# enoche/MMRec

Hardware: NVIDIA H100
Metric: graph-prop edges/sec (+ full-catalog scored-items/sec in extra) @ d=64 (higher is better)
Workload: dtype f32

## Files before the change

### mmrec_b200/csrc/score_cf.cu

```cuda
#include <climits>
#include <cstdio>
#include <cstdlib>

#include "batch_mask.cuh"
#include "select.cuh"
#include "tc_common.cuh"

namespace mmrec {

using namespace tc;

constexpr int CF_TILE = 128;
constexpr int CF_CONSUMER_WARPS = 8;
constexpr int CF_THREADS = 32 * CF_CONSUMER_WARPS + 32;
constexpr int CF_MAX_STAGES = 10;
constexpr int CF_CAP = 512;
constexpr int CF_EX_SLOTS = 128;
constexpr float CF_EPS = 1.125f / 1024.f;
constexpr float CF_EPS_SUB = 1.0f / 16777216.f;

struct CfSmem {
    uint32_t a, slab0, slab, bars, total;
    int stages;
};
__host__ __device__ inline CfSmem cf_smem(int KP) {
    CfSmem L;
    L.a = 0;
    L.slab0 = 2 * CF_TILE * KP * 2;
    const uint32_t slab = CF_TILE * KP * 2;
    L.slab = slab;
    L.stages = (int)((226u * 1024u - L.slab0 - 300u) / slab);
    if (L.stages > CF_MAX_STAGES) L.stages = CF_MAX_STAGES;
    L.bars = L.slab0 + L.stages * slab;
    L.total = L.bars + 32 * 8;
    return L;
}
enum { CB_AFULL = 0, CB_AFREE = 1, CB_FULL = 2, CB_EMPTY = 2 + CF_MAX_STAGES, CB_END = 2 + 2 * CF_MAX_STAGES };

struct CfParams {
    const char* Upk;
    const char* Ipk;
    int KP, n_it;
    int64_t B, n_items, n_units;
    float* gmax; int G, gw;
    const float* thr; uint4* bitmap;
    int dbg;
};

__device__ __forceinline__ void cf_producer(const CfParams& p, const CfSmem& L, uint32_t sbase, int64_t u0, int64_t u1) {
    const uint32_t bar = sbase + L.bars;
    const uint32_t a_bytes = 2 * CF_TILE * p.KP * 2;
    const uint32_t piece = L.slab < 16384u ? L.slab : 16384u;
    int64_t pair = u0 / p.n_it;
    int it = (int)(u0 - pair * p.n_it);
    bool new_pair = true;
    uint32_t a_cnt = 0, slot = 0, ph = 1;
    for (int64_t u = u0; u < u1; ++u) {
        if (new_pair) {
            if (a_cnt > 0) mbar_wait(bar + CB_AFREE * 8, (a_cnt - 1) & 1);
            mbar_expect_tx(bar + CB_AFULL * 8, a_bytes);
            const char* src = p.Upk + pair * (int64_t)a_bytes;
            for (uint32_t o = 0; o < a_bytes; o += 16384) bulk_g2s(sbase + L.a + o, src + o, 16384, bar + CB_AFULL * 8);
            ++a_cnt;
            new_pair = false;
        }
        const char* src = p.Ipk + (int64_t)it * L.slab;
        const uint32_t fb = bar + (CB_FULL + slot) * 8;
        mbar_wait(bar + (CB_EMPTY + slot) * 8, ph);
        if (p.dbg & 16) {
            mbar_arrive(fb);
        } else {
            mbar_expect_tx(fb, L.slab);
            const uint32_t dst = sbase + L.slab0 + slot * L.slab;
            for (uint32_t o = 0; o < L.slab; o += piece) bulk_g2s(dst + o, src + o, piece, fb);
        }
        if (++slot == (uint32_t)L.stages) { slot = 0; ph ^= 1; }
        if (++it == p.n_it) { it = 0; ++pair; new_pair = true; }
    }
}

template <int PASS, int GPT>
__device__ __forceinline__ void cf_consumer(const CfParams& p, const CfSmem& L, uint32_t sbase, int64_t u0, int64_t u1, int h) {
    const uint32_t bar = sbase + L.bars;
    constexpr uint32_t LBO = (CF_TILE / 8) * 128, SBO = 128;
    const int ksteps = p.KP / 16;
    const uint32_t half_bytes = CF_TILE * p.KP * 2;
    const int t = threadIdx.x & 127, w = t >> 5, lane = t & 31, q = lane & 3;
    const uint64_t a_desc0 = smem_desc(sbase + L.a + h * half_bytes, LBO, SBO), a_desc1 = smem_desc(sbase + L.a + h * half_bytes + 1024, LBO, SBO);
    const uint64_t b_desc0 = smem_desc(sbase + L.slab0, LBO, SBO);
    const uint64_t kstep = (2 * LBO) >> 4;
    const uint64_t slab_step = L.slab >> 4;
    float acc0[64], acc1[64];
#pragma unroll
    for (int i = 0; i < 64; ++i) { acc0[i] = 0.f; acc1[i] = 0.f; }
    int64_t pair = u0 / p.n_it;
    int it = (int)(u0 - pair * p.n_it);
    bool new_pair = true, live = false;
    uint32_t a_cnt = 0, slot = 0, ph = 0;
    uint64_t bd_slot = b_desc0;
    int64_t row0 = 0;
    float thr[4];
    for (int64_t u = u0; u < u1; ++u) {
        if (new_pair) {
            mbar_wait(bar + CB_AFULL * 8, a_cnt & 1);
            ++a_cnt;
            const int64_t base = pair * (2 * CF_TILE) + h * CF_TILE;
            live = base < p.B;
            row0 = base + 16 * w + (lane >> 2);
#pragma unroll
            for (int r = 0; r < 4; ++r) {
                const int64_t rr = row0 + 64 * (r >> 1) + 8 * (r & 1);
                if (PASS == 2) thr[r] = rr < p.B ? __ldg(p.thr + rr) : INFINITY;
            }
            new_pair = false;
        }
        mbar_wait(bar + (CB_FULL + slot) * 8, ph);
        if (live && !(p.dbg & 2)) {
            uint64_t ad0 = a_desc0, ad1 = a_desc1, bd = bd_slot;
            wgmma_fence();
#pragma unroll 4
            for (int j = 0; j < ksteps; ++j) {
                wgmma_f16<CF_TILE>(acc0, ad0, bd, j ? 1u : 0u);
                wgmma_f16<CF_TILE>(acc1, ad1, bd, j ? 1u : 0u);
                ad0 += kstep; ad1 += kstep; bd += kstep;
            }
            wgmma_commit();
            wgmma_wait<0>();
            wgmma_fence_regs(acc0);
            wgmma_fence_regs(acc1);
        }
        warp_arrive(bar + (CB_EMPTY + slot) * 8);
        bd_slot += slab_step;
        if (++slot == (uint32_t)L.stages) { slot = 0; ph ^= 1; bd_slot = b_desc0; }
        const int cur_it = it;
        if (++it == p.n_it) { it = 0; ++pair; new_pair = true; }
        if (new_pair || u + 1 == u1) warp_arrive(bar + CB_AFREE * 8);
        if (!live) continue;
        const int n_valid = (int)(p.n_items - (int64_t)cur_it * CF_TILE);
#pragma unroll
        for (int r = 0; r < 4; ++r) {
            const float* acc = r < 2 ? acc0 : acc1;
            const int e2 = r & 1;
            const int64_t row = row0 + 64 * (r >> 1) + 8 * e2;
            auto val = [&](int j, int e) {
                const float v = acc[4 * j + 2 * e2 + e];
                return 8 * j + 2 * q + e < n_valid ? v : -INFINITY;
            };
            if (PASS == 1) {
                group_max_store<GPT>(r < 2 ? acc0 : acc1, e2, q, n_valid, row, p.B, [&] { return p.gmax + row * p.G + (int64_t)cur_it * GPT; });
            } else {
                uint32_t wd[4] = {0u, 0u, 0u, 0u};
#pragma unroll
                for (int j = 0; j < 16; ++j)
#pragma unroll
                    for (int e = 0; e < 2; ++e)
                        if (!(__float_as_uint(val(j, e) - thr[r]) >> 31)) wd[j >> 2] |= 1u << (31 - (8 * (j & 3) + 2 * q + e));
#pragma unroll
                for (int b = 0; b < 4; ++b) {
                    wd[b] |= __shfl_xor_sync(0xffffffffu, wd[b], 1);
                    wd[b] |= __shfl_xor_sync(0xffffffffu, wd[b], 2);
                }
                if (q == r && row < p.B) p.bitmap[row * p.n_it + cur_it] = make_uint4(wd[0], wd[1], wd[2], wd[3]);
            }
        }
    }
}

template <int PASS, int GPT>
__global__ void __launch_bounds__(CF_THREADS, 1) cf_pass_kernel(const CfParams p) {
    extern __shared__ __align__(1024) uint8_t smem[];
    const CfSmem L = cf_smem(p.KP);
    const uint32_t sbase = smem_u32(smem);
    const int warp = threadIdx.x >> 5, lane = threadIdx.x & 31;
    const uint32_t bar = sbase + L.bars;
    if (threadIdx.x == 0) {
        mbar_init(bar + CB_AFULL * 8, 1);
        mbar_init(bar + CB_AFREE * 8, CF_CONSUMER_WARPS);
        for (int s = 0; s < CF_MAX_STAGES; ++s) {
            mbar_init(bar + (CB_FULL + s) * 8, 1);
            mbar_init(bar + (CB_EMPTY + s) * 8, CF_CONSUMER_WARPS);
        }
        mbar_fence_init();
    }
    __syncthreads();
    const int64_t u0 = (int64_t)blockIdx.x * p.n_units / gridDim.x;
    const int64_t u1 = (int64_t)(blockIdx.x + 1) * p.n_units / gridDim.x;
    if (warp == CF_CONSUMER_WARPS) {
        if (lane == 0) cf_producer(p, L, sbase, u0, u1);
    } else {
        cf_consumer<PASS, GPT>(p, L, sbase, u0, u1, warp >> 2);
    }
}

__device__ __forceinline__ void cf_pack_one(int64_t t, int64_t n_rows, const int64_t* __restrict__ idx, const float* __restrict__ E, int64_t ld,
                                            int d, int KP, const uint32_t* __restrict__ scale_src, uint4* __restrict__ out,
                                            float* __restrict__ row_norm, uint32_t* __restrict__ max_norm) {
    const int kblks = KP / 8;
    const int64_t row = t / kblks;
    const int kb = (int)(t % kblks);
    float x[8];
#pragma unroll
    for (int e = 0; e < 8; ++e) x[e] = 0.f;
    if (row < n_rows) {
        const float* src = E + (idx ? idx[row] : row) * ld;
#pragma unroll
        for (int e = 0; e < 8; ++e)
            if (kb * 8 + e < d) x[e] = __ldg(src + kb * 8 + e);
    }
    uint32_t am = 0u;
    if (!scale_src) {
#pragma unroll
        for (int e = 0; e < 8; ++e) { const uint32_t b = __float_as_uint(x[e]) & 0x7fffffffu; am = b > am ? b : am; }
        for (int o = kblks / 2; o > 0; o >>= 1) {
            const uint32_t a2 = __shfl_xor_sync(0xffffffffu, am, o);
            am = a2 > am ? a2 : am;
        }
    }
    const float sc = fp16_scale_for(scale_src ? __ldg(scale_src) : am);
    float ss = 0.f;
#pragma unroll
    for (int e = 0; e < 8; ++e) ss = fmaf(x[e] * sc, x[e] * sc, ss);
    for (int o = kblks / 2; o > 0; o >>= 1) ss += __shfl_xor_sync(0xffffffffu, ss, o);
    store_fp16x8(out, row / CF_TILE, kblks, kb, (int)(row % CF_TILE), x, sc);
    if (kb == 0 && row < n_rows) {
        const float nrm = sqrtf(ss) * (1.0f + 1e-6f);
        if (row_norm) row_norm[row] = nrm;
        if (max_norm) atomicMax(max_norm, __float_as_uint(nrm));
    }
}

__global__ void __launch_bounds__(256) cf_pack_items_kernel(int64_t n_items, const float* __restrict__ Ie, int64_t ldi, int d, int KP,
                                                            uint4* __restrict__ Ipk, uint32_t* __restrict__ header, int64_t n_threads) {
    const int64_t t = blockIdx.x * (int64_t)blockDim.x + threadIdx.x;
    if (t >= n_threads) return;
    if (t == 0) { header[1] = (uint32_t)n_items; header[2] = (uint32_t)d; header[3] = (uint32_t)KP; }
    cf_pack_one(t, n_items, nullptr, Ie, ldi, d, KP, header + 4, Ipk, nullptr, header);
}

__global__ void __launch_bounds__(256) cf_prep_kernel(int64_t mask_blocks, const BatchMask mask, int64_t nb, const int64_t* __restrict__ users,
                                                      const float* __restrict__ Ue, int64_t ldu, int d, int KP, uint4* __restrict__ Upk,
                                                      float* __restrict__ unorm, int64_t pack_threads, uint32_t* __restrict__ zero, int64_t zero_words) {
    if ((int64_t)blockIdx.x < mask_blocks) {
        mask_sorted_block(blockIdx.x, mask);
        return;
    }
    int64_t t = (blockIdx.x - mask_blocks) * (int64_t)blockDim.x + threadIdx.x;
    if (t < pack_threads) { cf_pack_one(t, nb, users, Ue, ldu, d, KP, nullptr, Upk, unorm, nullptr); return; }
    t -= pack_threads;
    if (t < zero_words) zero[t] = 0;
}

constexpr int CF_THR_BITS = 16;
template <int NV>
__device__ __forceinline__ uint32_t cf_warp_kth_coarse(const float* __restrict__ g, int G, int need, int lane) {
    uint32_t key[NV];
#pragma unroll
    for (int j = 0; j < NV; ++j) {
        const int t = j * 32 + lane;
        key[j] = t < G ? float_key(__ldg(g + t)) : 0u;
    }
    uint32_t kmax = 0u, kmin = 0xffffffffu;
#pragma unroll
    for (int j = 0; j < NV; ++j) {
        kmax = max(kmax, key[j]);
        if (j * 32 + lane < G && key[j] > 0x007fffffu) kmin = min(kmin, key[j]);
    }
    kmax = __reduce_max_sync(0xffffffffu, kmax);
    kmin = __reduce_min_sync(0xffffffffu, kmin);
    const int top = 31 - __clz((kmax ^ kmin) | (1u << (32 - CF_THR_BITS)));
    uint32_t prefix = top >= 31 ? 0u : (kmax & ~((2u << top) - 1u));
#pragma unroll 1
    for (int b = top; b >= 32 - CF_THR_BITS; --b) {
        const uint32_t cand = prefix | (1u << b);
        int cnt = 0;
#pragma unroll
        for (int j = 0; j < NV; ++j) cnt += key[j] >= cand;
        cnt = __reduce_add_sync(0xffffffffu, cnt);
        if (cnt >= need) prefix = cand;
    }
    return prefix;
}

__global__ void __launch_bounds__(256) cf_thr_kernel(int64_t nb, int G, int G_valid, int k, int d, const float* __restrict__ gmax, const float* __restrict__ unorm,
                                                     const uint32_t* __restrict__ max_norm, const int32_t* __restrict__ mask_ptr,
                                                     float* __restrict__ thr, int32_t* __restrict__ flags) {
    __shared__ RadixSmem radix_all[8];
    const int lane = threadIdx.x & 31, warp = threadIdx.x >> 5;
    const int64_t row = (int64_t)blockIdx.x * 8 + warp;
    if (row >= nb) return;
    const int need = k + (mask_ptr ? mask_ptr[row + 1] - mask_ptr[row] : 0);
    if (need > G_valid) {
        if (lane == 0) { thr[row] = INFINITY; flags[row] = 1; }
        return;
    }
    const float* g = gmax + row * G;
    uint32_t kth;
    if (G <= 16 * 32) kth = cf_warp_kth_coarse<16>(g, G, need, lane);
    else if (G <= 32 * 32) kth = cf_warp_kth_coarse<32>(g, G, need, lane);
    else {
        unsigned need_u = (unsigned)need;
        kth = radix_select<4, 32>([=](int64_t t) { return float_key(__ldg(g + t)); }, G, need_u, radix_all[warp]);
    }
    if (lane == 0) {
        const float un = unorm[row], mn = __uint_as_float(*max_norm);
        set_threshold(key_float(kth), 2.0f * (CF_EPS * un * mn + CF_EPS_SUB * sqrtf((float)d) * (un + mn + 1.0f)), thr + row, flags + row);
    }
}

__host__ __device__ constexpr int cf_lpr(int d) { return d <= 32 ? 8 : (d <= 64 ? 16 : 32); }

__device__ __forceinline__ float4 cf_load4(const float* __restrict__ row, int l, int d, bool vec_ok) {
    float4 x = make_float4(0.f, 0.f, 0.f, 0.f);
    if (vec_ok) {
        if (4 * l < d) x = ldg4(row + 4 * l);
    } else {
        if (4 * l < d) x.x = __ldg(row + 4 * l);
        if (4 * l + 1 < d) x.y = __ldg(row + 4 * l + 1);
        if (4 * l + 2 < d) x.z = __ldg(row + 4 * l + 2);
        if (4 * l + 3 < d) x.w = __ldg(row + 4 * l + 3);
    }
    return x;
}
__device__ __forceinline__ float cf_chain4(const float4 u, const float4 x) {
    return fmaf(u.w, x.w, fmaf(u.z, x.z, fmaf(u.y, x.y, fmaf(u.x, x.x, 0.f))));
}

template <int LPR>
__device__ __forceinline__ float cf_dot_thread_t(const float* __restrict__ u_sm , const float* __restrict__ v, int d, bool vec_ok) {
    float p[LPR];
#pragma unroll
    for (int l0 = 0; l0 < LPR; l0 += 8) {
        float4 x[8];
#pragma unroll
        for (int i = 0; i < 8; ++i) x[i] = cf_load4(v, l0 + i, d, vec_ok);
#pragma unroll
        for (int i = 0; i < 8; ++i) p[l0 + i] = cf_chain4(*reinterpret_cast<const float4*>(u_sm + 4 * (l0 + i)), x[i]);
    }
#pragma unroll
    for (int w = LPR / 2; w >= 1; w >>= 1)
#pragma unroll
        for (int a = 0; a < w; ++a) p[a] = p[a] + p[a + w];
    return p[0];
}
__device__ __forceinline__ float cf_dot_thread(const float* __restrict__ u_sm, const float* __restrict__ v, int d, bool vec_ok) {
    return d <= 32 ? cf_dot_thread_t<8>(u_sm, v, d, vec_ok) : (d <= 64 ? cf_dot_thread_t<16>(u_sm, v, d, vec_ok) : cf_dot_thread_t<32>(u_sm, v, d, vec_ok));
}

template <int LPR>
__device__ __forceinline__ float cf_dot_round(const float4 uu, const float* __restrict__ Ie, int64_t ldi, int d, bool vec_ok,
                                              const int32_t* cand, int t0, int n, int lane) {
    constexpr int RPI = 32 / LPR, NI = LPR;
    const int l = lane & (LPR - 1), sub = lane / LPR;
    float p[NI];
#pragma unroll
    for (int h = 0; h < NI; h += 8) {
        float4 x[8];
#pragma unroll
        for (int i = 0; i < 8; ++i) {
            const int t = t0 + (h + i) * RPI + sub;
            const int item = t < n ? cand[t] : -1;
            x[i] = make_float4(0.f, 0.f, 0.f, 0.f);
            if (item >= 0) x[i] = cf_load4(Ie + (int64_t)item * ldi, l, d, vec_ok);
        }
#pragma unroll
        for (int i = 0; i < 8; ++i) p[h + i] = cf_chain4(uu, x[i]);
    }
#pragma unroll
    for (int w = LPR / 2; w >= 1; w >>= 1) {
        const bool up = (l & w) != 0;
#pragma unroll
        for (int a = 0; a < w; ++a) {
            const float keep = up ? p[a + w] : p[a];
            const float send = up ? p[a] : p[a + w];
            p[a] = keep + __shfl_xor_sync(0xffffffffu, send, w);
        }
    }
    return p[0];
}

template <int E>
__device__ __forceinline__ void cf_rank_sweeps(const int32_t* cand, const uint32_t* keys, int n, int kept, int k, int lane, int64_t row,
                                               int64_t item_offset, int64_t* __restrict__ out_idx, float* __restrict__ out_val) {
    for (int e0 = 0; e0 * 32 < n; e0 += E) {
        uint32_t mk[E];
        int rk[E];
#pragma unroll
        for (int e = 0; e < E; ++e) { const int t = (e0 + e) * 32 + lane; mk[e] = t < n ? keys[t] : 0u; rk[e] = 0; }
        int u2 = 0;
        for (; u2 + 8 <= n; u2 += 8) {
            uint32_t ku[8];
#pragma unroll
            for (int i = 0; i < 8; ++i) ku[i] = keys[u2 + i];
#pragma unroll
            for (int i = 0; i < 8; ++i)
#pragma unroll
                for (int e = 0; e < E; ++e) rk[e] += ku[i] > mk[e];
        }
        for (; u2 < n; ++u2) {
            const uint32_t ku = keys[u2];
#pragma unroll
            for (int e = 0; e < E; ++e) rk[e] += ku > mk[e];
        }
        bool tie = n > 32 * E;
        if (!tie) {
            int sr = 0;
#pragma unroll
            for (int e = 0; e < E; ++e) sr += mk[e] != 0u ? rk[e] : 0;
            tie = __reduce_add_sync(0xffffffffu, sr) != kept * (kept - 1) / 2;
        }
        if (tie) {
            for (int u2 = 0; u2 < n; ++u2) {
                const uint32_t ku = keys[u2];
#pragma unroll
                for (int e = 0; e < E; ++e) rk[e] += (ku == mk[e]) && (u2 < (e0 + e) * 32 + lane);
            }
        }
#pragma unroll
        for (int e = 0; e < E; ++e) {
            if (mk[e] != 0u && rk[e] < k) {
                out_idx[row * k + rk[e]] = (int64_t)cand[(e0 + e) * 32 + lane] + item_offset;
                out_val[row * k + rk[e]] = key_float(mk[e]);
            }
        }
    }
}

constexpr int CF_FIN_WARPS = 4;
template <int LPR>
__global__ void __launch_bounds__(32 * CF_FIN_WARPS, LPR <= 16 ? 8 : 6) cf_final_kernel(int64_t nb, int n_it, int64_t n_items, int d, int k, int64_t item_offset,
                                                                     const uint4* __restrict__ bitmap, const int64_t* __restrict__ users,
                                                                     const float* __restrict__ Ue, int64_t ldu, const float* __restrict__ Ie, int64_t ldi,
                                                                     const int32_t* __restrict__ mask_ptr, const int32_t* __restrict__ mask_items,
                                                                     int32_t* __restrict__ flags, int32_t* __restrict__ counter,
                                                                     int32_t* __restrict__ row_of_slot, int64_t* __restrict__ out_idx,
                                                                     float* __restrict__ out_val) {
    __shared__ int32_t cand_all[CF_FIN_WARPS][CF_CAP];
    __shared__ uint32_t key_all[CF_FIN_WARPS][CF_CAP];
    const int lane = threadIdx.x & 31, warp = threadIdx.x >> 5;
    const int64_t row = (int64_t)blockIdx.x * CF_FIN_WARPS + warp;
    if (row >= nb) return;
    auto condemn = [&](int why) {
        if (lane == 0) {
            if (why) flags[row] = why;
            row_of_slot[atomicAdd(counter, 1)] = (int32_t)row;
        }
    };
    const int flagged = __ldg(flags + row);
    const int m0 = mask_ptr ? __ldg(mask_ptr + row) : 0, m1 = mask_ptr ? __ldg(mask_ptr + row + 1) : 0;
    const int64_t urow = users ? __ldg(users + row) : row;
    const uint4* bm = bitmap + row * n_it;
    uint4 b0 = make_uint4(0u, 0u, 0u, 0u);
    if (lane < n_it) b0 = __ldg(bm + lane);
    if (flagged) { condemn(0); return; }
    int32_t* cand = cand_all[warp];
    uint32_t* keys = key_all[warp];
    int n = 0;
    for (int w0 = 0; w0 < n_it; w0 += 32) {
        const int wi = w0 + lane;
        uint4 b = b0;
        if (w0 > 0) { b = make_uint4(0u, 0u, 0u, 0u); if (wi < n_it) b = __ldg(bm + wi); }
        const int mine = __popc(b.x) + __popc(b.y) + __popc(b.z) + __popc(b.w);
        int incl = mine;
#pragma unroll
        for (int o = 1; o < 32; o <<= 1) {
            const int v = __shfl_up_sync(0xffffffffu, incl, o);
            if (lane >= o) incl += v;
        }
        int pos = n + incl - mine;
        n += __shfl_sync(0xffffffffu, incl, 31);
        if (mine) {
            const uint32_t ws[4] = {b.x, b.y, b.z, b.w};
#pragma unroll
            for (int q = 0; q < 4; ++q) {
                uint32_t x = ws[q];
                while (x) {
                    const int j = __clz(x);
                    x &= ~(0x80000000u >> j);
                    if (pos < CF_CAP) { cand[pos] = wi * CF_TILE + q * 32 + j; keys[pos] = 1u; }
                    ++pos;
                }
            }
        }
    }
    if (n > CF_CAP) { condemn(4); return; }
    __syncwarp();
    for (int q0 = m0; q0 < m1; q0 += 32) {
        const int q = q0 + lane;
        if (q < m1) {
            const int item = __ldg(mask_items + q);
            int lo = 0, hi = n;
            while (lo < hi) {
                const int mid = (lo + hi) >> 1;
                if (cand[mid] < item) lo = mid + 1; else hi = mid;
            }
            if (lo < n && cand[lo] == item) keys[lo] = 0u;
        }
    }
    __syncwarp();
    for (int t = lane; t < n; t += 32)
        if (keys[t] == 0u || cand[t] >= n_items) cand[t] |= (int32_t)0x80000000;
    __syncwarp();
    const bool vec_ok = (ldi & 3) == 0 && (d & 3) == 0 && ((((uintptr_t)Ie) & 15) == 0);
    const bool vec_u = (ldu & 3) == 0 && (d & 3) == 0 && ((((uintptr_t)Ue) & 15) == 0);
    const float4 uu = cf_load4(Ue + urow * ldu, lane & (LPR - 1), d, vec_u);
    int kept = 0;
    for (int t0 = 0; t0 < n; t0 += 32) {
        const float sc = cf_dot_round<LPR>(uu, Ie, ldi, d, vec_ok, cand, t0, n, lane);
        const int t = t0 + (lane & (LPR - 1)) * (32 / LPR) + lane / LPR;
        if (t < n) {
            const uint32_t key = cand[t] >= 0 ? float_key(sc) : 0u;
            kept += key != 0u;
            keys[t] = key;
        }
    }
    kept = __reduce_add_sync(0xffffffffu, kept);
    __syncwarp();
    if (kept < k) { condemn(8); return; }
    if (n <= 64) cf_rank_sweeps<2>(cand, keys, n, kept, k, lane, row, item_offset, out_idx, out_val);
    else if (n <= 96) cf_rank_sweeps<3>(cand, keys, n, kept, k, lane, row, item_offset, out_idx, out_val);
    else cf_rank_sweeps<4>(cand, keys, n, kept, k, lane, row, item_offset, out_idx, out_val);
}

__global__ void __launch_bounds__(256) cf_exact_kernel(const int64_t* __restrict__ users, const float* __restrict__ Ue, int64_t ldu,
                                                       int64_t n_items, const float* __restrict__ Ie, int64_t ldi, int d, int k,
                                                       int64_t item_offset, const int32_t* __restrict__ mask_ptr,
                                                       const int32_t* __restrict__ mask_items, const int32_t* __restrict__ counter,
                                                       const int32_t* __restrict__ row_of_slot, unsigned* __restrict__ keys_all,
                                                       int64_t* __restrict__ out_idx, float* __restrict__ out_val) {
    __shared__ TopkSmem sm;
    __shared__ __align__(16) float u_ex[128];
    const int n_flagged = *counter;
    const int tid = threadIdx.x;
    unsigned* keys = keys_all + (int64_t)blockIdx.x * n_items;
    for (int fr = blockIdx.x; fr < n_flagged; fr += gridDim.x) {
        const int64_t row = row_of_slot[fr];
        __syncthreads();
        const float* u = Ue + (users ? users[row] : row) * ldu;
        if (tid < 128) u_ex[tid] = tid < d ? u[tid] : 0.f;
        __syncthreads();
        const bool vec_ok = (ldi & 3) == 0 && (d & 3) == 0 && ((((uintptr_t)Ie) & 15) == 0);
        for (int64_t i = tid; i < n_items; i += 256) keys[i] = float_key(cf_dot_thread(u_ex, Ie + i * ldi, d, vec_ok));
        __syncthreads();
        const int m0 = mask_ptr ? mask_ptr[row] : 0, m1 = mask_ptr ? mask_ptr[row + 1] : 0;
        for (int q = m0 + tid; q < m1; q += 256) {
            const int64_t item = mask_items[q];
            if (item >= 0 && item < n_items) keys[item] = float_key(-1e10f);
        }
        __syncthreads();
        cta_topk_from_keys<256>([=](int64_t i) { return keys[i]; }, n_items, k, item_offset, out_idx + row * k, out_val + row * k, sm);
    }
}

static inline int cf_kp(int d) { return d <= 32 ? 32 : (d <= 64 ? 64 : 128); }
static inline int cf_gw(int64_t n_items) { return n_items <= 16384 ? 1 : (n_items <= 32768 ? 2 : (n_items <= 65536 ? 4 : 8)); }

constexpr size_t CF_CAT_HEADER = 1024;

size_t cf_catalog_bytes(int64_t n_items, int d) {
    if (n_items <= 0 || d < 1 || d > 128) return 0;
    const int64_t n_it = (n_items + CF_TILE - 1) / CF_TILE;
    return CF_CAT_HEADER + (size_t)n_it * CF_TILE * cf_kp(d) * 2;
}

int cf_catalog_pack(int64_t n_items, const float* Ie, int64_t ldi, int d, void* cat, size_t cat_bytes, cudaStream_t stream) {
    const size_t need = cf_catalog_bytes(n_items, d);
    if (!need || !cat || cat_bytes < need || (((uintptr_t)cat) & 1023)) { set_error("catalog_pack: bad shape, or buffer null / not 1024-byte aligned / smaller than mmrec_catalog_bytes"); return MMREC_EINVAL; }
    const int KP = cf_kp(d);
    const int64_t n_it = (n_items + CF_TILE - 1) / CF_TILE;
    MMREC_CUDA(cudaMemsetAsync(cat, 0, CF_CAT_HEADER, stream));
    {
        const int64_t blocks = (n_items + 7) / 8;
        absmax_norm_kernel<<<(unsigned)(blocks < 2368 ? blocks : 2368), 256, 0, stream>>>(n_items, Ie, ldi, d, nullptr, (uint32_t*)cat + 4, nullptr);
        MMREC_LAUNCH_CHECK();
    }
    const int64_t threads = n_it * CF_TILE * (KP / 8);
    cf_pack_items_kernel<<<(unsigned)((threads + 255) / 256), 256, 0, stream>>>(n_items, Ie, ldi, d, KP, (uint4*)((char*)cat + CF_CAT_HEADER),
                                                                                  (uint32_t*)cat, threads);
    MMREC_LAUNCH_CHECK();
    return MMREC_OK;
}

struct CfPlan {
    int KP, gw, G;
    int64_t n_it, rows_blk, rows_pad, n_pairs;
    size_t off_cat, off_upk, off_unorm, off_gmax, off_thr, off_bitmap, off_flags, off_mask, off_keys, total;
};

static CfPlan cf_plan(int64_t B, int64_t n_items, int d, int64_t mask_nnz, bool with_cat) {
    CfPlan P;
    P.KP = cf_kp(d);
    P.gw = cf_gw(n_items);
    P.n_it = (n_items + CF_TILE - 1) / CF_TILE;
    P.G = (int)(P.n_it * (8 / P.gw));
    const int64_t per_row = (int64_t)P.G * 4 + P.n_it * 16;
    int64_t rb = (512ll << 20) / per_row / (2 * CF_TILE) * (2 * CF_TILE);
    if (rb < 2 * CF_TILE) rb = 2 * CF_TILE;
    if (rb > 65536) rb = 65536;
    P.rows_blk = B < rb ? B : rb;
    P.rows_pad = (P.rows_blk + 2 * CF_TILE - 1) / (2 * CF_TILE) * (2 * CF_TILE);
    P.n_pairs = P.rows_pad / (2 * CF_TILE);
    size_t off = 0;
    auto take = [&](size_t bytes) { size_t o = off; off += align_up(bytes, 1024); return o; };
    P.off_cat = take(with_cat ? cf_catalog_bytes(n_items, d) : 0);
    P.off_upk = take((size_t)P.rows_pad * P.KP * 2);
    P.off_unorm = take((size_t)P.rows_pad * 4);
    P.off_gmax = take((size_t)P.rows_blk * P.G * 4);
    P.off_thr = take((size_t)P.rows_pad * 4);
    P.off_bitmap = take((size_t)P.rows_blk * P.n_it * 16);
    P.off_flags = take((size_t)(2 * P.rows_blk + 2) * 4);
    P.off_mask = take(batch_mask(nullptr, mask_nnz, nullptr, nullptr, B, 0, 0).bytes);
    P.off_keys = take((size_t)CF_EX_SLOTS * n_items * 4);
    P.total = off + 1024;
    return P;
}

bool score_cf_supported(int64_t B, int64_t n_items, int d, int k) {
    if (!(B > 0 && d >= 1 && d <= 128 && k >= 1 && k <= 256 && n_items < (1ll << 31))) return false;
    const int64_t G = (n_items + CF_TILE - 1) / CF_TILE * (8 / cf_gw(n_items));
    return G >= 2 * (int64_t)k;
}

size_t score_cf_workspace_bytes(int64_t B, int64_t n_items, int d, int k, int64_t mask_nnz, bool with_cat) {
    if (!score_cf_supported(B, n_items, d, k)) return 0;
    return cf_plan(B, n_items, d, mask_nnz, with_cat).total;
}

static cudaEvent_t g_cf_ev[10];
static int g_cf_nev = 0, g_cf_timing = -1;
static inline void cf_mark(cudaStream_t stream) {
    if (g_cf_timing <= 0 || g_cf_nev >= 10) return;
    if (!g_cf_ev[g_cf_nev]) cudaEventCreate(&g_cf_ev[g_cf_nev]);
    cudaEventRecord(g_cf_ev[g_cf_nev++], stream);
}
int score_cf_timing(float* us, int cap) {
    int n = 0;
    for (int i = 0; i + 1 < g_cf_nev && n < cap; ++i) {
        cudaEventSynchronize(g_cf_ev[i + 1]);
        float ms = 0.f;
        cudaEventElapsedTime(&ms, g_cf_ev[i], g_cf_ev[i + 1]);
        us[n++] = ms * 1000.f;
    }
    return n;
}

int score_cf(int64_t B, const int64_t* users, const float* Ue, int64_t ldu, int64_t n_items, const float* Ie, int64_t ldi,
             int d, const void* cat, int64_t mask_nnz, const int64_t* mask_rows, const int64_t* mask_cols, int k, int64_t item_offset,
             int64_t* out_idx, float* out_val, void* ws, size_t ws_bytes, cudaStream_t stream) {
    if (!score_cf_supported(B, n_items, d, k) || !ws) return 0;
    const CfPlan P = cf_plan(B, n_items, d, mask_nnz, cat == nullptr);
    char* base = (char*)(((uintptr_t)ws + 1023) & ~(uintptr_t)1023);
    if (ws_bytes < P.total + (size_t)(base - (char*)ws)) return 0;
    if (int rc = set_smem_once<cf_pass_kernel<1, 8>, cf_pass_kernel<1, 4>, cf_pass_kernel<1, 2>, cf_pass_kernel<1, 1>, cf_pass_kernel<2, 8>>(227 * 1024))
        return rc;
    if (g_cf_timing < 0) g_cf_timing = getenv("MMREC_CF_TIMING") ? 1 : 0;
    g_cf_nev = 0;
    cf_mark(stream);
    if (!cat) {
        int rc = cf_catalog_pack(n_items, Ie, ldi, d, base + P.off_cat, cf_catalog_bytes(n_items, d), stream);
        if (rc) return rc;
        cat = base + P.off_cat;
    }
    cf_mark(stream);
    const uint32_t* max_norm = (const uint32_t*)cat;
    const char* Ipk = (const char*)cat + CF_CAT_HEADER;
    uint4* Upk = (uint4*)(base + P.off_upk);
    float *unorm = (float*)(base + P.off_unorm), *gmax = (float*)(base + P.off_gmax), *thr = (float*)(base + P.off_thr);
    uint4* bitmap = (uint4*)(base + P.off_bitmap);
    int32_t* flags = (int32_t*)(base + P.off_flags);
    int32_t* counter = flags + P.rows_blk;
    int32_t* row_of_slot = counter + 1;
    const BatchMask M = batch_mask(base + P.off_mask, mask_nnz, mask_rows, mask_cols, B, item_offset, n_items);
    unsigned* keys = (unsigned*)(base + P.off_keys);
    constexpr int T = MC_SORTED_THREADS;
    const bool has_mask = mask_nnz > 0;
    const bool small_mask = has_mask && mask_small(B, mask_nnz);
    if (has_mask && !small_mask) {
        int rc = batch_mask_large(M, stream);
        if (rc) return rc;
    }
    const CfSmem L = cf_smem(P.KP);
    const int sms = sm_count();
    for (int64_t r0 = 0; r0 < B; r0 += P.rows_blk) {
        const int64_t nb = (B - r0) < P.rows_blk ? (B - r0) : P.rows_blk;
        const int64_t nb_pad = (nb + 2 * CF_TILE - 1) / (2 * CF_TILE) * (2 * CF_TILE);
        const int64_t n_pairs = nb_pad / (2 * CF_TILE);
        const int64_t* ub = users ? users + r0 : nullptr;
        const float* ue = users ? Ue : Ue + r0 * ldu;
        const int32_t* mp = has_mask ? M.ptr + r0 : nullptr;
        const int64_t mask_blocks = (small_mask && r0 == 0) ? mask_sorted_blocks(mask_nnz) : 0;
        const int64_t pack_threads = nb_pad * (P.KP / 8);
        const int64_t zero_words = P.rows_blk + 1;
        cf_prep_kernel<<<(unsigned)(mask_blocks + (pack_threads + zero_words + T - 1) / T), T, 0, stream>>>(
            mask_blocks, M, nb, ub, ue, ldu, d, P.KP, Upk, unorm, pack_threads, (uint32_t*)flags, zero_words);
        MMREC_LAUNCH_CHECK();
        if (mask_blocks) {
            int rc = batch_mask_unsorted(M, stream);
            if (rc) return rc;
        }
        cf_mark(stream);
        CfParams p;
        p.Upk = (const char*)Upk; p.Ipk = Ipk; p.KP = P.KP; p.n_it = (int)P.n_it; p.B = nb; p.n_items = n_items; p.n_units = n_pairs * P.n_it;
        p.gmax = gmax; p.G = P.G; p.gw = P.gw; p.thr = thr; p.bitmap = bitmap;
        { static int dbg = -1; if (dbg < 0) { const char* e = getenv("MMREC_CF_DEBUG"); dbg = e ? atoi(e) : 0; } p.dbg = dbg; }
        const unsigned grid = (unsigned)(p.n_units < sms ? p.n_units : sms);
        switch (P.gw) {
            case 1: cf_pass_kernel<1, 8><<<grid, CF_THREADS, L.total, stream>>>(p); break;
            case 2: cf_pass_kernel<1, 4><<<grid, CF_THREADS, L.total, stream>>>(p); break;
            case 4: cf_pass_kernel<1, 2><<<grid, CF_THREADS, L.total, stream>>>(p); break;
            default: cf_pass_kernel<1, 1><<<grid, CF_THREADS, L.total, stream>>>(p); break;
        }
        MMREC_LAUNCH_CHECK();
        cf_mark(stream);
        cf_thr_kernel<<<(unsigned)((nb + 7) / 8), 256, 0, stream>>>(nb, P.G, (int)((n_items + 16 * P.gw - 1) / (16 * P.gw)), k, d, gmax, unorm, max_norm, mp, thr, flags);
        MMREC_LAUNCH_CHECK();
        cf_mark(stream);
        cf_pass_kernel<2, 8><<<grid, CF_THREADS, L.total, stream>>>(p);
        MMREC_LAUNCH_CHECK();
        cf_mark(stream);
        {
            const unsigned fg = (unsigned)((nb + CF_FIN_WARPS - 1) / CF_FIN_WARPS);
#define CF_FINAL(LPR) cf_final_kernel<LPR><<<fg, 32 * CF_FIN_WARPS, 0, stream>>>(nb, (int)P.n_it, n_items, d, k, item_offset, bitmap, ub, ue, ldu, Ie, ldi, mp, \
                                                                            M.items, flags, counter, row_of_slot, out_idx + r0 * k, out_val + r0 * k)
            if (cf_lpr(d) == 8) CF_FINAL(8); else if (cf_lpr(d) == 16) CF_FINAL(16); else CF_FINAL(32);
#undef CF_FINAL
        }
        MMREC_LAUNCH_CHECK();
        cf_mark(stream);
        cf_exact_kernel<<<CF_EX_SLOTS, 256, 0, stream>>>(ub, ue, ldu, n_items, Ie, ldi, d, k, item_offset, mp, M.items, counter, row_of_slot, keys,
                                                         out_idx + r0 * k, out_val + r0 * k);
        MMREC_LAUNCH_CHECK();
        cf_mark(stream);
    }
    return 1;
}

int64_t score_cf_fallback_rows(const void* ws, int64_t B, int64_t n_items, int d, int k, int64_t mask_nnz, bool with_cat) {
    if (!score_cf_supported(B, n_items, d, k) || !ws) return -1;
    const CfPlan P = cf_plan(B, n_items, d, mask_nnz, with_cat);
    const char* base = (const char*)(((uintptr_t)ws + 1023) & ~(uintptr_t)1023);
    int32_t n = 0;
    if (cudaMemcpy(&n, base + P.off_flags + (size_t)P.rows_blk * 4, 4, cudaMemcpyDeviceToHost) != cudaSuccess) return -1;
    if (getenv("MMREC_DEBUG")) {
        const int64_t nb = B % P.rows_blk ? B % P.rows_blk : P.rows_blk;
        int32_t* h = (int32_t*)malloc((size_t)nb * 4);
        if (h && cudaMemcpy(h, base + P.off_flags, (size_t)nb * 4, cudaMemcpyDeviceToHost) == cudaSuccess) {
            long long why[4] = {0, 0, 0, 0};
            for (int64_t i = 0; i < nb; ++i)
                for (int b = 0; b < 4; ++b) why[b] += (h[i] >> b) & 1;
            fprintf(stderr, "mmrec: exact-path rows %d of %lld (need > groups %lld, non-finite %lld, > %d candidates %lld, < k kept %lld)\n", n,
                    (long long)nb, why[0], why[1], CF_CAP, why[2], why[3]);
        }
        free(h);
    }
    return n;
}

}
```

### mmrec_b200/csrc/tc_common.cuh

```cuda
#pragma once
#include <cuda_fp16.h>

#include "common.cuh"
#include "wgmma.cuh"

namespace mmrec {
namespace tc {

__device__ __forceinline__ uint32_t smem_u32(const void* p) { return (uint32_t)__cvta_generic_to_shared(p); }

__device__ __forceinline__ void mbar_init(uint32_t bar, uint32_t count) {
    asm volatile("mbarrier.init.shared::cta.b64 [%0], %1;" ::"r"(bar), "r"(count) : "memory");
}
__device__ __forceinline__ void mbar_fence_init() { asm volatile("fence.mbarrier_init.release.cluster;" ::: "memory"); }
__device__ __forceinline__ void mbar_arrive(uint32_t bar) {
    asm volatile("mbarrier.arrive.shared::cta.b64 _, [%0];" ::"r"(bar) : "memory");
}
__device__ __forceinline__ void mbar_expect_tx(uint32_t bar, uint32_t bytes) {
    asm volatile("mbarrier.arrive.expect_tx.shared::cta.b64 _, [%0], %1;" ::"r"(bar), "r"(bytes) : "memory");
}
__device__ __forceinline__ bool mbar_try_wait(uint32_t bar, uint32_t parity) {
    uint32_t ok;
    asm volatile(
        "{\n\t.reg .pred p;\n\t"
        "mbarrier.try_wait.parity.shared::cta.b64 p, [%1], %2;\n\t"
        "selp.u32 %0, 1, 0, p;\n\t}"
        : "=r"(ok) : "r"(bar), "r"(parity) : "memory");
    return ok != 0;
}
__device__ __forceinline__ uint64_t global_ns() {
    uint64_t t;
    asm volatile("mov.u64 %0, %%globaltimer;" : "=l"(t));
    return t;
}
__device__ __forceinline__ void mbar_wait(uint32_t bar, uint32_t parity) {
    uint32_t spins = 0;
    uint64_t t0 = 0;
    while (!mbar_try_wait(bar, parity)) {
        if (++spins == 4096u) t0 = global_ns();
        if (spins > 4096u && (spins & 1023u) == 0 && global_ns() - t0 > 2000000000ull) __trap();
    }
}

__device__ __forceinline__ void bulk_g2s(uint32_t dst_smem, const void* src, uint32_t bytes, uint32_t bar) {
    asm volatile("cp.async.bulk.shared::cluster.global.mbarrier::complete_tx::bytes [%0], [%1], %2, [%3];"
                 ::"r"(dst_smem), "l"(src), "r"(bytes), "r"(bar) : "memory");
}

__device__ __forceinline__ void wgmma_fence() { asm volatile("wgmma.fence.sync.aligned;" ::: "memory"); }
__device__ __forceinline__ void wgmma_commit() { asm volatile("wgmma.commit_group.sync.aligned;" ::: "memory"); }
template <int N>
__device__ __forceinline__ void wgmma_wait() { asm volatile("wgmma.wait_group.sync.aligned %0;" ::"n"(N) : "memory"); }
template <int R>
__device__ __forceinline__ void wgmma_fence_regs(float (&d)[R]) {
#pragma unroll
    for (int i = 0; i < R; ++i) asm volatile("" : "+f"(d[i])::"memory");
}
__device__ __forceinline__ void fence_proxy_async() { asm volatile("fence.proxy.async.shared::cta;" ::: "memory"); }
__device__ __forceinline__ void warp_arrive(uint32_t bar) {
    __syncwarp();
    if ((threadIdx.x & 31) == 0) mbar_arrive(bar);
}

__device__ __forceinline__ uint64_t smem_desc(uint32_t smem_addr, uint32_t lbo_bytes, uint32_t sbo_bytes) {
    uint64_t d = 0;
    d |= (uint64_t)((smem_addr & 0x3FFFFu) >> 4);
    d |= (uint64_t)((lbo_bytes >> 4) & 0x3FFFu) << 16;
    d |= (uint64_t)((sbo_bytes >> 4) & 0x3FFFu) << 32;
    return d;
}

__device__ __forceinline__ void split_tf32(float x, float& hi, float& lo) {
    uint32_t h, l;
    asm("cvt.rna.tf32.f32 %0, %1;" : "=r"(h) : "f"(x));
    hi = __uint_as_float(h);
    asm("cvt.rna.tf32.f32 %0, %1;" : "=r"(l) : "f"(x - hi));
    lo = __uint_as_float(l);
}

__device__ __forceinline__ void split_tf32_trunc(float x, float& hi, float& lo) {
    hi = __uint_as_float(__float_as_uint(x) & 0xffffe000u);
    lo = x - hi;
}

}

__device__ __forceinline__ float fp16_scale_for(uint32_t m_bits) {
    const uint32_t e = (m_bits >> 23) & 0xffu;
    if (e == 0u || e == 255u || e < 14u) return 1.0f;
    return __uint_as_float((268u - e) << 23);
}

__global__ void absmax_norm_kernel(int64_t n, const float* __restrict__ X, int64_t ldx, int F, float* __restrict__ rnorm,
                                   uint32_t* __restrict__ amax, uint32_t* __restrict__ nmax);

__device__ __forceinline__ void store_fp16x8(uint4* __restrict__ out, int64_t tile, int kblks, int kb, int rr, const float (&x)[8], float sc) {
    uint32_t w[4];
#pragma unroll
    for (int e = 0; e < 4; ++e) {
        const __half2 h = __floats2half2_rn(x[2 * e] * sc, x[2 * e + 1] * sc);
        w[e] = *reinterpret_cast<const uint32_t*>(&h);
    }
    out[((tile * kblks + kb) * 16 + rr / 8) * 8 + (rr % 8)] = make_uint4(w[0], w[1], w[2], w[3]);
}

template <int GPT, class Dst>
__device__ __forceinline__ void group_max_store(const float (&acc)[64], int e2, int q, int n_valid, int64_t row, int64_t n_rows, Dst dst) {
    auto val = [&](int j, int e) { return 8 * j + 2 * q + e < n_valid ? acc[4 * j + 2 * e2 + e] : -INFINITY; };
    float gm[GPT];
#pragma unroll
    for (int g = 0; g < GPT; ++g) {
        float m = -INFINITY;
#pragma unroll
        for (int j = g * (16 / GPT); j < (g + 1) * (16 / GPT); ++j) m = fmaxf(m, fmaxf(val(j, 0), val(j, 1)));
        m = fmaxf(m, __shfl_xor_sync(0xffffffffu, m, 1));
        gm[g] = fmaxf(m, __shfl_xor_sync(0xffffffffu, m, 2));
    }
    if (row < n_rows) {
        float* d = dst();
#pragma unroll
        for (int g = 0; g < GPT; ++g)
            if ((g & 3) == q) d[g] = gm[g];
    }
}

__device__ __forceinline__ void set_threshold(float t, float margin, float* thr, int32_t* flag) {
    const bool finite = fabsf(t) < INFINITY && margin < INFINITY;
    *thr = finite ? t - margin : INFINITY;
    *flag = finite ? 0 : 2;
}

constexpr int TC_M = 128;
constexpr int TC_N = 256;
constexpr int TC_KC = 32;
constexpr int TC_SLAB_BYTES = TC_N * TC_KC * 4;
constexpr int TC_THREADS = 288;

template <int R>
__device__ __forceinline__ void pack_split_one(int64_t t, int64_t n_rows, const int64_t* __restrict__ idx, const float* __restrict__ E,
                                               int64_t ld, int d, int KP, float* __restrict__ hi, float* __restrict__ lo) {
    const int kblks = KP / 4;
    const int64_t row = t / kblks;
    const int kb = (int)(t % kblks);
    float x[4] = {0.f, 0.f, 0.f, 0.f};
    if (row < n_rows) {
        const float* src = E + (idx ? idx[row] : row) * ld;
#pragma unroll
        for (int e = 0; e < 4; ++e)
            if (kb * 4 + e < d) x[e] = __ldg(src + kb * 4 + e);
    }
    float4 h, l;
    tc::split_tf32(x[0], h.x, l.x); tc::split_tf32(x[1], h.y, l.y); tc::split_tf32(x[2], h.z, l.z); tc::split_tf32(x[3], h.w, l.w);
    const int64_t tile = row / R;
    const int rr = (int)(row % R);
    const int64_t off = ((tile * kblks + kb) * (R / 8) + rr / 8) * 32 + (rr % 8) * 4;
    *reinterpret_cast<float4*>(hi + off) = h;
    *reinterpret_cast<float4*>(lo + off) = l;
}

template <int R>
__global__ void pack_split_kernel(int64_t n_rows, const int64_t* __restrict__ idx, const float* __restrict__ E, int64_t ld,
                                  int d, int KP, float* __restrict__ hi, float* __restrict__ lo, int64_t n_tiles) {
    const int64_t t = blockIdx.x * (int64_t)blockDim.x + threadIdx.x;
    if (t >= n_tiles * R * (KP / 4)) return;
    pack_split_one<R>(t, n_rows, idx, E, ld, d, KP, hi, lo);
}

}
```

Measured before the change: 13.68 billion.

## Ping-pong consumer warpgroups with token barriers, register rebalancing, and specialized epilogue

```diff
diff --git a/mmrec_b200/csrc/score_cf.cu b/mmrec_b200/csrc/score_cf.cu
--- a/mmrec_b200/csrc/score_cf.cu
+++ b/mmrec_b200/csrc/score_cf.cu
@@ -12,7 +12,7 @@
 
 constexpr int CF_TILE = 128;
 constexpr int CF_CONSUMER_WARPS = 8;
-constexpr int CF_THREADS = 32 * CF_CONSUMER_WARPS + 32;
+constexpr int CF_THREADS = 32 * CF_CONSUMER_WARPS + 128;
 constexpr int CF_MAX_STAGES = 10;
 constexpr int CF_CAP = 512;
 constexpr int CF_EX_SLOTS = 128;
@@ -35,7 +35,8 @@
     L.total = L.bars + 32 * 8;
     return L;
 }
-enum { CB_AFULL = 0, CB_AFREE = 1, CB_FULL = 2, CB_EMPTY = 2 + CF_MAX_STAGES, CB_END = 2 + 2 * CF_MAX_STAGES };
+enum { CB_AFULL = 0, CB_AFREE = 1, CB_FULL = 2, CB_EMPTY = 2 + CF_MAX_STAGES, CB_TOK = 2 + 2 * CF_MAX_STAGES, CB_END = CB_TOK + 2 };
+static_assert(CB_END <= 32, "cf_smem reserves 32 barrier slots");
 
 struct CfParams {
     const char* Upk;
@@ -79,12 +80,50 @@
     }
 }
 
-template <int PASS, int GPT>
+template <int PASS, int GPT, bool TAIL>
+__device__ __forceinline__ void cf_epilogue(const CfParams& p, const float (&acc0)[64], const float (&acc1)[64], const float (&thr)[4],
+                                            int64_t row0, int q, int cur_it, int n_valid) {
+#pragma unroll
+    for (int r = 0; r < 4; ++r) {
+        const float(&acc)[64] = r < 2 ? acc0 : acc1;
+        const int e2 = r & 1;
+        const int64_t row = row0 + 64 * (r >> 1) + 8 * e2;
+        if (PASS == 1) {
+            group_max_store<GPT, TAIL>(acc, e2, q, n_valid, row, p.B, [&] { return p.gmax + row * p.G + (int64_t)cur_it * GPT; });
+        } else {
+            uint32_t wd[4];
+#pragma unroll
+            for (int b = 0; b < 4; ++b) {
+                uint32_t w = 0u;
+#pragma unroll
+                for (int jj = 0; jj < 4; ++jj) {
+                    if (jj) w <<= 6;
+#pragma unroll
+                    for (int e = 0; e < 2; ++e) {
+                        const int j = 4 * b + jj;
+                        float v = acc[4 * j + 2 * e2 + e];
+                        if (TAIL && 8 * j + 2 * q + e >= n_valid) v = -INFINITY;
+                        w = __funnelshift_l(__float_as_uint(__fsub_rn(v, thr[r])), w, 1);
+                    }
+                }
+                wd[b] = w << (6 - 2 * q);
+            }
+#pragma unroll
+            for (int b = 0; b < 4; ++b) {
+                wd[b] |= __shfl_xor_sync(0xffffffffu, wd[b], 1);
+                wd[b] = ~(wd[b] | __shfl_xor_sync(0xffffffffu, wd[b], 2));
+            }
+            if (q == r && row < p.B) p.bitmap[row * p.n_it + cur_it] = make_uint4(wd[0], wd[1], wd[2], wd[3]);
+        }
+    }
+}
+
+template <int PASS, int GPT, int KP>
 __device__ __forceinline__ void cf_consumer(const CfParams& p, const CfSmem& L, uint32_t sbase, int64_t u0, int64_t u1, int h) {
     const uint32_t bar = sbase + L.bars;
     constexpr uint32_t LBO = (CF_TILE / 8) * 128, SBO = 128;
-    const int ksteps = p.KP / 16;
-    const uint32_t half_bytes = CF_TILE * p.KP * 2;
+    constexpr int ksteps = KP / 16;
+    constexpr uint32_t half_bytes = CF_TILE * KP * 2;
     const int t = threadIdx.x & 127, w = t >> 5, lane = t & 31, q = lane & 3;
     const uint64_t a_desc0 = smem_desc(sbase + L.a + h * half_bytes, LBO, SBO), a_desc1 = smem_desc(sbase + L.a + h * half_bytes + 1024, LBO, SBO);
     const uint64_t b_desc0 = smem_desc(sbase + L.slab0, LBO, SBO);
@@ -96,10 +135,11 @@
     int64_t pair = u0 / p.n_it;
     int it = (int)(u0 - pair * p.n_it);
     bool new_pair = true, live = false;
-    uint32_t a_cnt = 0, slot = 0, ph = 0;
+    uint32_t a_cnt = 0, slot = 0, ph = 0, tok_ph = 0;
     uint64_t bd_slot = b_desc0;
     int64_t row0 = 0;
     float thr[4];
+    const uint32_t tok_wait = bar + (CB_TOK + h) * 8, tok_pass = bar + (CB_TOK + (h ^ 1)) * 8;
     for (int64_t u = u0; u < u1; ++u) {
         if (new_pair) {
             mbar_wait(bar + CB_AFULL * 8, a_cnt & 1);
@@ -115,20 +155,23 @@
             new_pair = false;
         }
         mbar_wait(bar + (CB_FULL + slot) * 8, ph);
-        if (live && !(p.dbg & 2)) {
+        if (h == 1 || u > u0) { mbar_wait(tok_wait, tok_ph); tok_ph ^= 1; }
+        const bool mma = live && !(p.dbg & 2);
+        if (mma) {
             uint64_t ad0 = a_desc0, ad1 = a_desc1, bd = bd_slot;
             wgmma_fence();
-#pragma unroll 4
+#pragma unroll
             for (int j = 0; j < ksteps; ++j) {
                 wgmma_f16<CF_TILE>(acc0, ad0, bd, j ? 1u : 0u);
                 wgmma_f16<CF_TILE>(acc1, ad1, bd, j ? 1u : 0u);
                 ad0 += kstep; ad1 += kstep; bd += kstep;
             }
             wgmma_commit();
-            wgmma_wait<0>();
-            wgmma_fence_regs(acc0);
-            wgmma_fence_regs(acc1);
-        }
+        }
+        warp_arrive(tok_pass);
+        wgmma_wait<0>();
+        wgmma_fence_regs(acc0);
+        wgmma_fence_regs(acc1);
         warp_arrive(bar + (CB_EMPTY + slot) * 8);
         bd_slot += slab_step;
         if (++slot == (uint32_t)L.stages) { slot = 0; ph ^= 1; bd_slot = b_desc0; }
@@ -137,39 +180,15 @@
         if (new_pair || u + 1 == u1) warp_arrive(bar + CB_AFREE * 8);
         if (!live) continue;
         const int n_valid = (int)(p.n_items - (int64_t)cur_it * CF_TILE);
-#pragma unroll
-        for (int r = 0; r < 4; ++r) {
-            const float* acc = r < 2 ? acc0 : acc1;
-            const int e2 = r & 1;
-            const int64_t row = row0 + 64 * (r >> 1) + 8 * e2;
-            auto val = [&](int j, int e) {
-                const float v = acc[4 * j + 2 * e2 + e];
-                return 8 * j + 2 * q + e < n_valid ? v : -INFINITY;
-            };
-            if (PASS == 1) {
-                group_max_store<GPT>(r < 2 ? acc0 : acc1, e2, q, n_valid, row, p.B, [&] { return p.gmax + row * p.G + (int64_t)cur_it * GPT; });
-            } else {
-                uint32_t wd[4] = {0u, 0u, 0u, 0u};
-#pragma unroll
-                for (int j = 0; j < 16; ++j)
-#pragma unroll
-                    for (int e = 0; e < 2; ++e)
-                        if (!(__float_as_uint(val(j, e) - thr[r]) >> 31)) wd[j >> 2] |= 1u << (31 - (8 * (j & 3) + 2 * q + e));
-#pragma unroll
-                for (int b = 0; b < 4; ++b) {
-                    wd[b] |= __shfl_xor_sync(0xffffffffu, wd[b], 1);
-                    wd[b] |= __shfl_xor_sync(0xffffffffu, wd[b], 2);
-                }
-                if (q == r && row < p.B) p.bitmap[row * p.n_it + cur_it] = make_uint4(wd[0], wd[1], wd[2], wd[3]);
-            }
-        }
-    }
-}
-
-template <int PASS, int GPT>
+        if (n_valid >= CF_TILE) cf_epilogue<PASS, GPT, false>(p, acc0, acc1, thr, row0, q, cur_it, n_valid);
+        else cf_epilogue<PASS, GPT, true>(p, acc0, acc1, thr, row0, q, cur_it, n_valid);
+    }
+}
+
+template <int PASS, int GPT, int KP>
 __global__ void __launch_bounds__(CF_THREADS, 1) cf_pass_kernel(const CfParams p) {
     extern __shared__ __align__(1024) uint8_t smem[];
-    const CfSmem L = cf_smem(p.KP);
+    const CfSmem L = cf_smem(KP);
     const uint32_t sbase = smem_u32(smem);
     const int warp = threadIdx.x >> 5, lane = threadIdx.x & 31;
     const uint32_t bar = sbase + L.bars;
@@ -180,15 +199,19 @@
             mbar_init(bar + (CB_FULL + s) * 8, 1);
             mbar_init(bar + (CB_EMPTY + s) * 8, CF_CONSUMER_WARPS);
         }
+        mbar_init(bar + CB_TOK * 8, CF_CONSUMER_WARPS / 2);
+        mbar_init(bar + (CB_TOK + 1) * 8, CF_CONSUMER_WARPS / 2);
         mbar_fence_init();
     }
     __syncthreads();
     const int64_t u0 = (int64_t)blockIdx.x * p.n_units / gridDim.x;
     const int64_t u1 = (int64_t)(blockIdx.x + 1) * p.n_units / gridDim.x;
-    if (warp == CF_CONSUMER_WARPS) {
-        if (lane == 0) cf_producer(p, L, sbase, u0, u1);
+    if (warp >= CF_CONSUMER_WARPS) {
+        asm volatile("setmaxnreg.dec.sync.aligned.u32 40;\n" ::: "memory");
+        if (warp == CF_CONSUMER_WARPS && lane == 0) cf_producer(p, L, sbase, u0, u1);
     } else {
-        cf_consumer<PASS, GPT>(p, L, sbase, u0, u1, warp >> 2);
+        asm volatile("setmaxnreg.inc.sync.aligned.u32 232;\n" ::: "memory");
+        cf_consumer<PASS, GPT, KP>(p, L, sbase, u0, u1, warp >> 2);
     }
 }
 
@@ -643,6 +666,24 @@
     return n;
 }
 
+#define CF_PASS_KERNELS(KP) cf_pass_kernel<1, 8, KP>, cf_pass_kernel<1, 4, KP>, cf_pass_kernel<1, 2, KP>, cf_pass_kernel<1, 1, KP>, cf_pass_kernel<2, 8, KP>
+template <int PASS, int KP>
+static void cf_pass_launch_kp(int gw, unsigned grid, uint32_t smem, cudaStream_t stream, const CfParams& p) {
+    if (PASS == 2) { cf_pass_kernel<2, 8, KP><<<grid, CF_THREADS, smem, stream>>>(p); return; }
+    switch (gw) {
+        case 1: cf_pass_kernel<1, 8, KP><<<grid, CF_THREADS, smem, stream>>>(p); break;
+        case 2: cf_pass_kernel<1, 4, KP><<<grid, CF_THREADS, smem, stream>>>(p); break;
+        case 4: cf_pass_kernel<1, 2, KP><<<grid, CF_THREADS, smem, stream>>>(p); break;
+        default: cf_pass_kernel<1, 1, KP><<<grid, CF_THREADS, smem, stream>>>(p); break;
+    }
+}
+template <int PASS>
+static void cf_pass_launch(int KP, int gw, unsigned grid, uint32_t smem, cudaStream_t stream, const CfParams& p) {
+    if (KP == 32) cf_pass_launch_kp<PASS, 32>(gw, grid, smem, stream, p);
+    else if (KP == 64) cf_pass_launch_kp<PASS, 64>(gw, grid, smem, stream, p);
+    else cf_pass_launch_kp<PASS, 128>(gw, grid, smem, stream, p);
+}
+
 int score_cf(int64_t B, const int64_t* users, const float* Ue, int64_t ldu, int64_t n_items, const float* Ie, int64_t ldi,
              int d, const void* cat, int64_t mask_nnz, const int64_t* mask_rows, const int64_t* mask_cols, int k, int64_t item_offset,
              int64_t* out_idx, float* out_val, void* ws, size_t ws_bytes, cudaStream_t stream) {
@@ -650,8 +691,7 @@
     const CfPlan P = cf_plan(B, n_items, d, mask_nnz, cat == nullptr);
     char* base = (char*)(((uintptr_t)ws + 1023) & ~(uintptr_t)1023);
     if (ws_bytes < P.total + (size_t)(base - (char*)ws)) return 0;
-    if (int rc = set_smem_once<cf_pass_kernel<1, 8>, cf_pass_kernel<1, 4>, cf_pass_kernel<1, 2>, cf_pass_kernel<1, 1>, cf_pass_kernel<2, 8>>(227 * 1024))
-        return rc;
+    if (int rc = set_smem_once<CF_PASS_KERNELS(32), CF_PASS_KERNELS(64), CF_PASS_KERNELS(128)>(227 * 1024)) return rc;
     if (g_cf_timing < 0) g_cf_timing = getenv("MMREC_CF_TIMING") ? 1 : 0;
     g_cf_nev = 0;
     cf_mark(stream);
@@ -703,18 +743,13 @@
         p.gmax = gmax; p.G = P.G; p.gw = P.gw; p.thr = thr; p.bitmap = bitmap;
         { static int dbg = -1; if (dbg < 0) { const char* e = getenv("MMREC_CF_DEBUG"); dbg = e ? atoi(e) : 0; } p.dbg = dbg; }
         const unsigned grid = (unsigned)(p.n_units < sms ? p.n_units : sms);
-        switch (P.gw) {
-            case 1: cf_pass_kernel<1, 8><<<grid, CF_THREADS, L.total, stream>>>(p); break;
-            case 2: cf_pass_kernel<1, 4><<<grid, CF_THREADS, L.total, stream>>>(p); break;
-            case 4: cf_pass_kernel<1, 2><<<grid, CF_THREADS, L.total, stream>>>(p); break;
-            default: cf_pass_kernel<1, 1><<<grid, CF_THREADS, L.total, stream>>>(p); break;
-        }
+        cf_pass_launch<1>(P.KP, P.gw, grid, L.total, stream, p);
         MMREC_LAUNCH_CHECK();
         cf_mark(stream);
         cf_thr_kernel<<<(unsigned)((nb + 7) / 8), 256, 0, stream>>>(nb, P.G, (int)((n_items + 16 * P.gw - 1) / (16 * P.gw)), k, d, gmax, unorm, max_norm, mp, thr, flags);
         MMREC_LAUNCH_CHECK();
         cf_mark(stream);
-        cf_pass_kernel<2, 8><<<grid, CF_THREADS, L.total, stream>>>(p);
+        cf_pass_launch<2>(P.KP, P.gw, grid, L.total, stream, p);
         MMREC_LAUNCH_CHECK();
         cf_mark(stream);
         {
diff --git a/mmrec_b200/csrc/tc_common.cuh b/mmrec_b200/csrc/tc_common.cuh
--- a/mmrec_b200/csrc/tc_common.cuh
+++ b/mmrec_b200/csrc/tc_common.cuh
@@ -104,9 +104,9 @@
     out[((tile * kblks + kb) * 16 + rr / 8) * 8 + (rr % 8)] = make_uint4(w[0], w[1], w[2], w[3]);
 }
 
-template <int GPT, class Dst>
+template <int GPT, bool TAIL = true, class Dst>
 __device__ __forceinline__ void group_max_store(const float (&acc)[64], int e2, int q, int n_valid, int64_t row, int64_t n_rows, Dst dst) {
-    auto val = [&](int j, int e) { return 8 * j + 2 * q + e < n_valid ? acc[4 * j + 2 * e2 + e] : -INFINITY; };
+    auto val = [&](int j, int e) { return !TAIL || 8 * j + 2 * q + e < n_valid ? acc[4 * j + 2 * e2 + e] : -INFINITY; };
     float gm[GPT];
 #pragma unroll
     for (int g = 0; g < GPT; ++g) {
```

Result: no change. 13.72 billion, median of 6 (+0.2%).
